# AlmondGod/diffusion-piano

Hardware: AMD Instinct MI355X
Metric: env steps/sec at 4096 parallel envs; qpos L∞ drift vs CPU MuJoCo (higher is better)
Workload: dtype f32; 1 GPU; 4096 envs/GPU crossing_field random-action rollout, 10 physics substeps per env-step, constraint forces by the primal Newton solve (friction loss, uncapped rows); envs_per_gpu=4096, song=crossing_field, parallelism=dp1

## Files before the change

diffusion-piano_amd/csrc/devmodel.h:

```cpp
#pragma once
#include <stdint.h>

#include "../../include/pianosim.h"

namespace ps {

constexpr int NK = PS_NKEY;
constexpr int NH = PS_NHAND;
constexpr int NB = PS_HAND_NBODY;
constexpr int ND = PS_HAND_NDOF;
constexpr int NG = PS_HAND_NGEOM;
constexpr int NA = PS_HAND_NACT;
constexpr int NV = PS_NV;
constexpr int NU = PS_NU;
constexpr int NBT = NH * NB;
constexpr int NDT = NH * ND;
constexpr int NGT = NH * NG;
constexpr int NX = PS_HAND_NXGEOM;
constexpr int NXT = NH * NX;
constexpr int NCOLL = NGT + NXT;
static_assert(NCOLL <= 64, "one lane per collider");
constexpr int NTT = NH * PS_HAND_NTENDON;
constexpr int MAXDEP = 9;
constexpr int MAXLEV = 8;
constexpr int MAXCHILD = 5;
constexpr int MAXCON = 24;
constexpr int KEYLANE = 52;
constexpr int YS = 20;
constexpr int YKEY = 19;
constexpr int NTRI = MAXDEP * (MAXDEP - 1) / 2;
constexpr int NKB = 64;
constexpr int KGEO = 16;
constexpr int XCG = 4;
constexpr int XNCELL = 6 * XCG * XCG;
constexpr int XCV = 8;

struct DevModel {
  float timestep;
  int nsub;
  float grav[3];
  float hgrav[3];
  float key_pos[NK][3], key_half[NK][3], key_anchor[NK][3];
  float key_mass[NK], key_Minv[NK], key_Mhinv[NK], key_damp[NK], key_stiff[NK], key_sref[NK];
  float key_lo[NK], key_hi[NK], key_ylo[NK], key_yhi[NK], key_binv[NK], key_dinv[NK];
  float base_pos[3], base_half[3];
  float pc_solref[2], pc_solimp[5], pc_fric;
  float hc_solref[2], hc_solimp[5], hc_fric;
  float lim_solref[2], lim_solimp[5];
  float fr_solref[2], fr_solimp[5];
  int body_parent[NBT];
  float body_pos[NBT][3], body_Q[NBT][9], body_mass[NBT], body_ipos[NBT][3], body_I[NBT][6];
  float body_binv[NBT];
  int body_dof[NBT], body_ndof[NBT];
  uint64_t body_pathmask[NBT];
  int nlev, lev_start[MAXLEV + 1], lev_body[NBT];
// ... 3 lines not shown
  float dof_floss[NDT];
  int dof_depth[NDT], dof_anc[NDT][MAXDEP];
  uint64_t dof_ancmask[NDT];
  uint64_t dof_descmask[NDT];
  int dof_ndesc[NDT], dof_desc[NDT][ND];
  int ndepth, dep_start[MAXDEP + 1], dep_dof[NDT];
  int dof_act[NDT];
  float dof_act_coef[NDT];
  int obs_dof[NDT];
  int n_obsj;
  uint64_t dof_lockmask;
  int act_src[NU];
  int n_action;
  int act_kind[NU], act_dof0[NU], act_dof1[NU], act_flim[NU];
  float act_c0[NU], act_c1[NU], act_kp[NU], act_clo[NU], act_chi[NU], act_flo[NU], act_fhi[NU];
  int geom_body[NCOLL];
  uint64_t geom_pathmask[NCOLL];
  float geom_binv[NCOLL];
  float geom_pos[NGT][3], geom_axis[NGT][3], geom_hl[NGT], geom_r[NGT];
  int root_geom_count;
  int site_body[NH * PS_NFINGER];
  float site_pos[NH * PS_NFINGER][3];
  int npairs;
  int pair[PS_MAX_CAPPAIRS][2];
  int nx;
  int x_type[NXT];
  float x_pos[NXT][3], x_Q[NXT][9], x_hs[NXT][3], x_rb[NXT];
  int x_v0[NXT], x_nv[NXT];
  float x_ec[NXT][8];
  uint64_t x_cell[NXT][XNCELL];
  alignas(16) float x_cellv[NXT][XNCELL + 1][XCV][4];
  int x_cellv_ok[NXT];
  int nxpairs;
  int nxpairs_same;
  int xpair[PS_MAX_XPAIRS];
  alignas(16) float hull_v[NH * PS_HAND_HULLVERT][4];
  int tri_a[NTRI + 8], tri_b[NTRI + 8];
  int body_level[NBT];
  int body_child_pack[NBT];
  int dof_anc_pack[NDT][3];
  float key_top_zmax;
  float piano_xmin, piano_xmax;
  float kb_y0, kb_inv;
  uint8_t kb_first[NKB], kb_end[NKB];
  int npairs_same;
  alignas(16) float key_geo[NK][KGEO];
};

}
```

diffusion-piano_amd/csrc/kernel_v2.inc:

```

#ifdef PS_TIMING
#define NPHASE 56
#define TARG , uint64_t *tacc, uint64_t &tlast
#define TPASS , tacc, tlast
#define TSTAMP(slot)                                     \
  do {                                                   \
    __syncthreads();                                     \
    uint64_t t_ = __builtin_amdgcn_s_memtime();         \
    tacc[slot] += t_ - tlast;                            \
    tlast = t_;                                          \
  } while (0)
__device__ uint64_t* g_timing = nullptr;
#else
#define TSTAMP(slot) \
  do {               \
  } while (0)
#define TARG
#define TPASS
#endif

#ifdef PS_CHECK_A
__device__ int g_dbg_count = 0;
#endif
enum : int { BX_R = 0, BX_CP = 0, BX_O = 10, BX_W = 13, BX_AL = 16, BX_AC = 19, BX_F = 22, BX_N = 25, BXS = 28 };
static_assert(NKB == 64, "collide2 stages one key-range bucket per lane");
// ... 381 lines not shown
        cc.g2 = g2;
      }
    }
  }
  return rt;
}

constexpr int NSTAGE = 32, STAGE_OFF = 2 * 256;
static_assert(STAGE_OFF >= 2 * NSTAGE, "candidate list overlaps the staging area");
constexpr int CPL = 8, CSTAGE_OFF = 2 * NGT * CPL;

template <bool XG, int WPE>
__device__ __forceinline__ int collide2(const DevModel* __restrict__ m, Shared& S, int maxc, int lane, float c_r TARG) {
  static_assert(STAGE_OFF + 2 * NSTAGE * sizeof(Contact) <= sizeof(S.bx), "contact staging exceeds bx");
  static_assert(CSTAGE_OFF + 2 * 64 * CPL <= sizeof(S.bx), "candidate staging exceeds bx");
  const bool isc = lane < NGT;
  {
    const float4* src = reinterpret_cast<const float4*>(&m->key_geo[0][0]);
    float4* dst = reinterpret_cast<float4*>(&S.kg[0][0]);
    for (int i = lane; i < NK * KGEO / 4; i += 64) dst[i] = src[i];
    S.kb[0][lane] = m->kb_first[lane];
    S.kb[1][lane] = m->kb_end[lane];
  }
  wsync();
  uint16_t* cand = reinterpret_cast<uint16_t*>(&S.bx[0][0]);
  constexpr int MAXCAND = (int)(sizeof(S.bx) / sizeof(uint16_t));
  int ncand;
  {
    uint16_t* cst = reinterpret_cast<uint16_t*>(reinterpret_cast<char*>(&S.bx[0][0]) + CSTAGE_OFF) + lane * CPL;
    const int cnt = isc ? piano_candidates(m, S, lane, c_r, cst, CPL) : 0;
    const int off = small_excl_scan<7>(cnt, lane, &ncand);
    if (__ballot(cnt > CPL) == 0ull) {
      for (int j = 0; j < cnt; j++) cand[off + j] = cst[j];
    } else if (isc && cnt && off + cnt <= MAXCAND) {
      piano_candidates(m, S, lane, c_r, cand + off, cnt);
    }
    ncand = min(ncand, MAXCAND);
  }
  wsync();
  TSTAMP(11);
  int total = 0;
  if (ncand <= NSTAGE) {
    Contact* stage = reinterpret_cast<Contact*>(reinterpret_cast<char*>(&S.bx[0][0]) + STAGE_OFF);
    const int pr = lane < ncand ? (int)cand[lane] : 0;
    const int cnt = lane < ncand ? piano_pair<WPE>(m, S, pr, stage, 2 * lane, 2 * lane + 2) : 0;
    int rt;
// ... 4 lines not shown
    ncand = 0;
  }
  for (int r0 = 0; r0 < ncand && total < maxc; r0 += 64) {
    const int i = r0 + lane;
    const int pr = i < ncand ? (int)cand[i] : 0;
    const int cnt = i < ncand ? piano_pair<WPE>(m, S, pr, nullptr, 0, 0) : 0;
    int rt;
    const int off = small_excl_scan<2>(cnt, lane, &rt);
    if (cnt) piano_pair<WPE>(m, S, pr, S.con, total + off, maxc);
    total += rt;
  }
  TSTAMP(7);
  int base = total;
  float lo[3], hi[3];
  {
    f3 p0 = isc ? ld3(&S.cap[lane][0]) : mk3(0, 0, 0), p1 = isc ? ld3(&S.cap[lane][3]) : mk3(0, 0, 0);
    lo[0] = fminf(p0.x, p1.x) - c_r; lo[1] = fminf(p0.y, p1.y) - c_r; lo[2] = fminf(p0.z, p1.z) - c_r;
    hi[0] = fmaxf(p0.x, p1.x) + c_r; hi[1] = fmaxf(p0.y, p1.y) + c_r; hi[2] = fmaxf(p0.z, p1.z) + c_r;
  }
  bool inb = isc;
  int hb = lane < NG ? 0 : 1;
  if (XG && lane >= NGT) {
    const int e = lane - NGT;
    inb = m->x_type[e] != PS_GEOM_NONE;
    hb = e / NX;
    if (inb) {
      const f3 ctr = ld3(S.xg[e]);
      const float rb = m->x_rb[e];
      lo[0] = ctr.x - rb; lo[1] = ctr.y - rb; lo[2] = ctr.z - rb;
      hi[0] = ctr.x + rb; hi[1] = ctr.y + rb; hi[2] = ctr.z + rb;
    }
  }
  bool apart = false;
  {
#pragma unroll
    for (int i = 0; i < 3; i++) {
      const float l0 = wave_min(inb && hb == 0 ? lo[i] : INFINITY), l1 = wave_min(inb && hb == 1 ? lo[i] : INFINITY);
      const float h0 = -wave_min(inb && hb == 0 ? -hi[i] : INFINITY),
                  h1 = -wave_min(inb && hb == 1 ? -hi[i] : INFINITY);
      if (h0 < l1 || h1 < l0) apart = true;
    }
  }
  const int npairs = apart ? m->npairs_same : m->npairs;
  uint16_t* near = cand;
  int nnear = 0;
  int pnext = lane < npairs ? m->pair[lane][0] | (m->pair[lane][1] << 8) : 0;
  for (int p0 = 0; p0 < npairs; p0 += 64) {
    const int p = p0 + lane;
    const int pk = pnext;
    if (p0 + 64 < npairs) pnext = p + 64 < npairs ? m->pair[p + 64][0] | (m->pair[p + 64][1] << 8) : 0;
    bool pass = false;
    if (p < npairs) {
      const float* A = S.cap[pk & 255];
      const float* B = S.cap[pk >> 8];
      const f3 ca = (ld3(A) + ld3(A + 3)) * 0.5f, cb = (ld3(B) + ld3(B + 3)) * 0.5f;
      pass = norm3(ca - cb) <= A[7] + B[7] + A[6] + B[6];
    }
    const uint64_t mask = __ballot(pass);
    if (pass) near[nnear + lanes_below(mask, lane)] = (uint16_t)pk;
    nnear += __popcll(mask);
  }
  wsync();
  for (int q0 = 0; q0 < nnear && base < maxc; q0 += 64) {
    const int q = q0 + lane;
    bool hit = false;
    f3 c1, c2;
    float ra = 0, rb = 0, dn = 0;
    int ga = 0, gb = 0;
    if (q < nnear) {
      const int pk = near[q];
      ga = pk & 255;
      gb = pk >> 8;
      const float* A = S.cap[ga];
      const float* B = S.cap[gb];
      ra = A[6];
      rb = B[6];
      seg_seg(ld3(A), ld3(A + 3), ld3(B), ld3(B + 3), &c1, &c2);
      dn = norm3(c2 - c1);
      hit = dn - ra - rb <= 0.f;
    }
    uint64_t mask = __ballot(hit);
    int slot = base + lanes_below(mask, lane);
    if (hit && slot < maxc) {
      Contact& cc = S.con[slot];
      f3 dv = c2 - c1;
      f3 n = dn > 1e-9f ? dv * (1.f / dn) : mk3(0, 0, 1);
      float dist = dn - ra - rb;
      st3(cc.n, n);
      cc.dist = dist;
      st3(cc.pos, c1 + n * (ra + 0.5f * dist));
      f3 t1, t2;
      make_frame(n, &t1, &t2);
      st3(cc.t1, t1); st3(cc.t2, t2);
      cc.kind = 2; cc.key = -1; cc.g1 = ga; cc.g2 = gb;
    }
    base += __popcll(mask);
  }
  if (XG && (m->nx || m->nxpairs)) {
    TSTAMP(2);
    int nl = 0;
    if (m->nx) {
      static_assert(NXT * CPL * 2 <= CSTAGE_OFF, "x candidates overlap the staging");
      const bool isx = lane >= NGT && m->x_type[lane >= NGT ? lane - NGT : 0] != PS_GEOM_NONE;
      uint16_t* cst = reinterpret_cast<uint16_t*>(reinterpret_cast<char*>(&S.bx[0][0]) + CSTAGE_OFF) + lane * CPL;
      wsync();
      const int cnt = isx ? xpiano_candidates(m, S, lane, cst, CPL) : 0;
      const int off = small_excl_scan<7>(cnt, lane, &nl);
      wsync();
      if (__ballot(cnt > CPL) == 0ull) {
        for (int j = 0; j < cnt; j++) cand[off + j] = cst[j];
      } else if (isx && cnt && off + cnt <= MAXCAND) {
        xpiano_candidates(m, S, lane, cand + off, cnt);
      }
      nl = min(nl, MAXCAND);
      wsync();
    }
    TSTAMP(32);
    if (m->nxpairs) {
      const int nxp = apart ? m->nxpairs_same : m->nxpairs;
      for (int p0 = 0; p0 < nxp; p0 += 64) {
        const int p = p0 + lane;
        bool pass = false;
        int pk = 0;
        if (p < nxp) {
          pk = m->xpair[p];
          const int ga = pk & 255, gb = pk >> 8;
          f3 c2[2];
          float rad = 0.f;
#pragma unroll
          for (int q = 0; q < 2; q++) {
            const int g = q ? gb : ga;
            if (g < NGT) {
              c2[q] = (ld3(&S.cap[g][0]) + ld3(&S.cap[g][3])) * 0.5f;
              rad += S.cap[g][6] + S.cap[g][7];
            } else {
              c2[q] = ld3(S.xg[g - NGT]);
              rad += m->x_rb[g - NGT];
            }
          }
          pass = norm3(c2[0] - c2[1]) <= rad;
        }
        const uint64_t mask = __ballot(pass);
        const int at = nl + lanes_below(mask, lane);
        if (pass && at < MAXCAND) cand[at] = (uint16_t)(pk | XHH);
        nl = min(nl + __popcll(mask), MAXCAND);
      }
#ifdef PS_TIMING
      tacc[45] += nl;
#endif
    }
    wsync();
    TSTAMP(35);
    nl = x_refine<WPE>(m, &S, cand, nl, lane);
#ifdef PS_TIMING
    tacc[42] += nl > 0;
#endif
    TSTAMP(36);
    for (int q0 = 0; q0 < nl && base < maxc; q0 += 32) {
      const int q = q0 + (lane >> 1);
      int ga, gb, key;
      x_entry(q < nl ? (int)cand[q] : 0, ga, gb, key);
#ifdef PS_TIMING
      int its[5] = {0, 0, 0, 0, 0};
      base += x_pairs<WPE>(m, &S, q < nl, ga, gb, key, S.con, base, maxc, lane, its);
      tacc[30] += its[0];
      tacc[31] += 1;
      tacc[38] += its[1];
      tacc[39] += its[2];
      tacc[40] += its[3];
      tacc[41] += its[4];
#else
      base += x_pairs<WPE>(m, &S, q < nl, ga, gb, key, S.con, base, maxc, lane);
#endif
    }
    TSTAMP(37);
  }
  if (lane == 0) S.ncon = base < maxc ? base : maxc;
  wsync();
  return base;
}

struct LaneStatic {
  int d_type, d_body, d_depth, d_ap0, d_ap1, d_act;
  uint64_t d_ancmask, d_desc;
  float d_axl[3], d_lo, d_hi, d_damp, d_arm, d_dinv, d_actc;
  bool d_lim;
  int b_parent, b_level, b_dof, b_ndof, b_chp, b_nch;
  int c_body;
  float c_r;
};

__device__ __forceinline__ void load_static(const DevModel* __restrict__ m, Shared& S, LaneStatic& L, int lane) {
  const int d = lane < NDT ? lane : 0, b = lane < NBT ? lane : 0, c = lane < NGT ? lane : 0;
  L.d_type = m->dof_type[d];
  L.d_body = m->dof_body[d];
  L.d_depth = lane < NDT ? m->dof_depth[d] : -1;
  L.d_ap0 = m->dof_anc_pack[d][0];
  L.d_ap1 = m->dof_anc_pack[d][1];
  L.d_act = m->dof_act[d];
  L.d_ancmask = m->dof_ancmask[d];
  L.d_desc = lane < NDT ? m->dof_descmask[d] : 0ull;
  for (int i = 0; i < 3; i++) L.d_axl[i] = m->dof_axis[d][i];
// ... 895 lines not shown
#pragma unroll
      for (int j = 0; j < 2; j++) {
        st_wt(pw + 64 * (CW_KQ + j), D.kq[j]);
        st_wt(pw + 64 * (CW_KV + j), D.kv[j]);
      }
      st_wt(pw + 64 * CW_CTRL, ctrl);
      st_wt(pw + 64 * CW_ACTF, actf_last);
      st_wt(pw + 64 * CW_ZF, __int_as_float(guess.zf));
      st_wt(pw + 64 * CW_ZL, __int_as_float(guess.zl));
      st_wt(pw + 64 * CW_ZC, __int_as_float(guess.zc));
      st_wt(pw + 64 * CW_CID, __int_as_float(guess.cid));
      st_wt(pw + 64 * CW_ZK, __int_as_float(guess.zk[0]));
      st_wt(pw + 64 * (CW_ZK + 1), __int_as_float(guess.zk[1]));
      const int sc = lane == CS_SOLVES ? st_solves : lane == CS_CONCAP ? st_concap : lane == CS_CAP ? st_cap
                   : lane == CS_MAXROW ? st_maxrow : lane == CS_COUPLED ? st_coupled : lane == CS_PIV ? st_piv
                   : lane == CS_CDOFS ? st_cdofs : lane == CS_WARN ? warn[0] : lane == CS_WARN + 1 ? warn[1]
                   : lane == CS_WARN + 2 ? warn[2] : lane == CS_GVALID ? (int)guess.valid
                   : (int)(bufs.applied && !applied);
      st_wt(pw + 64 * CW_SCAL, __int_as_float(sc));
      return true;
    }
  }
  kinematics2<false, XG>(m, S, L, D, lane, hand_dy TPASS);
  collide2<XG, WPE>(m, S, cfg.maxcon, lane, L.c_r TPASS);
  key_state2(m, S, D, lane);
  f3 root = mk3(0, 0, 0);
  if (cfg.hand) {
    const int B = (cfg.hand - 1) * NB;
    root = mk3(__shfl(D.o[0], B, 64), __shfl(D.o[1], B, 64), __shfl(D.o[2], B, 64));
  }
  if (do_reset) {
    write_obs2(m, song, cfg, S, 0, obs_e, lane, root);
    if (lane < NDT) {
      bufs.qpos[rowoff + NK + lane] = 0.f;
      bufs.qvel[rowoff + NK + lane] = 0.f;
      bufs.qws[rowoff + NK + lane] = 0.f;
    }
    for (int k = lane; k < NK; k += 64) {
      bufs.qpos[rowoff + k] = 0.f;
      bufs.qvel[rowoff + k] = 0.f;
      bufs.qws[rowoff + k] = 0.f;
    }
    if (lane < NU) bufs.ctrl[(size_t)e * NU + lane] = 0.f;
    if (lane < PS_NTERMS) bufs.terms[(size_t)e * PS_NTERMS + lane] = 0.f;
    if (lane < PS_NMUSIC) bufs.mus_acc[(size_t)e * PS_NMUSIC + lane] = 0.f;
    for (int s = 0; s < 2 * PS_NFINGER; s++) {
      f3 p = site_world2(m, D, s);
      if (lane == s) st3(bufs.tips + ((size_t)e * 2 * PS_NFINGER + s) * 3, p);
    }
    if (lane < PS_NSTATS) bufs.stats[(size_t)e * PS_NSTATS + lane] = 0;
    if (lane == 0) {
      bufs.sustain[e] = 0.f;
      bufs.t_idx[e] = 0;
      bufs.last[e] = 0;
      bufs.ncon[e] = S.ncon;
      if (bufs.keybits) bufs.keybits[(size_t)e * kb_stride(m->nsub)] = KB_NEW_EPISODE;
      if (mode == 0) {
        reward[e] = 0.f;
        discount[e] = 1.f;
        step_type[e] = PS_FIRST;
      }
    }
    return false;
  }
  const int t_cur = bufs.t_idx[e];
  const int t_new = t_cur + 1;
  const float* gc = song.goal + (size_t)t_cur * (NK + 1);
  float on_tol = 0.f, on_cnt = 0.f;
  bool fail_l = false;
  for (int k = lane; k < NK; k += 64) {
    float g = gc[k];
    bool act = (S.act_bits[k >> 5] >> (k & 31)) & 1;
    if (g != 0.f) { on_tol += tolerance(g - S.knorm[k], 0.f, 0.05f, 0.5f); on_cnt += 1.f; }
    else if (act) fail_l = true;
  }
  float sum_tol = wave_sum(on_tol), n_on = wave_sum(on_cnt);
  bool failure = __ballot(fail_l) != 0ull;
  float mus[PS_NMUSIC];
// ... 58 lines not shown
      if (on && pos < PS_MAX_NOTES) okeys[pos] = k;
      K += __popcll(mk);
    }
    K = min(K, PS_MAX_NOTES);
    wsync();
    float res = 1.f;
    if (K > 0) {
      for (int t0 = 0; t0 < 10 * K; t0 += 64) {
        const int t = t0 + lane;
        const int j = min(t / 10, K - 1), i = t - 10 * (t / 10);
        const int site = i < 5 ? PS_NFINGER + i : i - 5;
        const float tx = __shfl(tip_own.x, site, 64), ty = __shfl(tip_own.y, site, 64), tz = __shfl(tip_own.z, site, 64);
        const float dcost = norm3(key_target2(m, S, okeys[j]) - mk3(tx, ty, tz));
        if (t < 10 * K) ocost[K <= 10 ? j * 10 + i : i * K + j] = dcost < 1e30f ? dcost : 1e30f;
      }
      wsync();
      if (lane == 0) res = K <= 10 ? hungarian_tol(K, 10, ocost, owork) / K : hungarian_tol(10, K, ocost, owork) / 10.f;
    }
    fing = rdlane(res, 0);
  }
  float fore = 0.f;
  if (cfg.forearm) {
    bool hit = false;
    if (lane < S.ncon) {
      const Contact& cc = S.con[lane];
      if (cc.kind == 2) {
        const int b1 = m->geom_body[cc.g1], b2 = m->geom_body[cc.g2];
        hit = b1 % NB == 0 && b2 % NB == 0 && b1 != b2;
      }
    }
    fore = __ballot(hit) ? 0.f : 0.5f;
  }
  bool terminal = t_new == song.T;
  float disc = 1.f;
  if (!terminal && cfg.wrong_press && failure) { terminal = true; disc = 0.f; }
  write_obs2(m, song, cfg, S, t_new < song.T ? t_new : t_new - 1, obs_e, lane, root);
  if (lane < NDT) {
    bufs.qpos[rowoff + NK + lane] = D.q;
    bufs.qvel[rowoff + NK + lane] = D.v;
    bufs.qws[rowoff + NK + lane] = D.qws;
  }
#pragma unroll
  for (int j = 0; j < 2; j++) {
    int k = lane + 64 * j;
    if (k < NK) {
      bufs.qpos[rowoff + k] = D.kq[j];
      bufs.qvel[rowoff + k] = D.kv[j];
// ... 7 lines not shown
  if (lane < PS_NSTATS)
    bufs.stats[(size_t)e * PS_NSTATS + lane] = lane == 0 ? st_solves : lane == 1 ? st_concap : lane == 2 ? st_cap
                                               : lane == 3 ? st_maxrow : lane == 4 ? st_coupled
                                               : lane == 5 ? st_piv : st_cdofs;
  if (lane == 0) {
    float* tm = bufs.terms + (size_t)e * PS_NTERMS;
    tm[0] = kp; tm[1] = sus; tm[2] = energy; tm[3] = fing; tm[4] = fore;
    reward[e] = kp + sus + energy + fing + fore;
    discount[e] = disc;
    step_type[e] = terminal ? PS_LAST : PS_MID;
    float* ma = bufs.mus_acc + (size_t)e * PS_NMUSIC;
#pragma unroll
    for (int i = 0; i < PS_NMUSIC; i++) ma[i] += mus[i];
    if (terminal) {
      float* me = bufs.mus_ep + (size_t)e * PS_NMUSIC;
      const float inv = 1.f / (float)t_new;
#pragma unroll
      for (int i = 0; i < PS_NMUSIC; i++) me[i] = ma[i] * inv;
      bufs.mus_cnt[e] += 1;
    }
    bufs.sustain[e] = S.sustain;
    bufs.t_idx[e] = t_new;
    bufs.last[e] = terminal ? 1 : 0;
    bufs.ncon[e] = S.ncon;
    if (bufs.keybits) bufs.keybits[(size_t)e * kb_stride(m->nsub)] = (uint32_t)m->nsub;
  }
  if (bufs.con_out) {
    constexpr int CW = (int)(sizeof(Contact) / sizeof(int));
    const int* src = reinterpret_cast<const int*>(S.con);
    int* dst = reinterpret_cast<int*>(bufs.con_out) + (size_t)e * MAXCON * CW;
    for (int w = lane; w < S.ncon * CW; w += 64) dst[w] = src[w];
  }
#ifdef PS_TIMING
  TSTAMP(5);
  if (lane == 0 && g_timing)
    for (int i = 0; i < NPHASE; i++) g_timing[(size_t)e * NPHASE + i] += tacc[i];
#endif
  return false;
}

template <bool XG, int WPE = PS_WAVES_PER_EU>
__global__ void __launch_bounds__(64) __attribute__((amdgpu_waves_per_eu(WPE))) pianosim_kernel(const DevModel* __restrict__ m, Song song, Cfg cfg, Bufs bufs,
                                                      const float* __restrict__ action, const uint8_t* __restrict__ mask,
                                                      float* __restrict__ obs, float* __restrict__ reward,
                                                      float* __restrict__ discount, uint8_t* __restrict__ step_type,
                                                      int mode, int n_envs, const int* __restrict__ order) {
#ifdef PS_DYN_LDS
  extern __shared__ __attribute__((aligned(16))) char smem_[];
  Shared& S = *reinterpret_cast<Shared*>(smem_);
#else
  __shared__ Shared S;
#endif
  const int e = order ? order[blockIdx.x] : (int)blockIdx.x;
  const int lane = threadIdx.x;
  if (e >= n_envs) return;
  env_step<XG, WPE, false>(S, m, song, cfg, bufs, action, mask, obs, reward, discount, step_type, mode, e, lane, 0, 1);
}

enum : int { QC_HEAD = 0, QC_WORDS = 32 };
#ifndef PS_TIMING
enum : int { QE_NONE = -1, QE_LEFT = -2 };
struct QArgs {
  const DevModel* m;
  Song song;
  Cfg cfg;
  Bufs bufs;
  const float* action;
  float *obs, *reward, *discount;
  uint8_t* step_type;
  int n_envs;
  int *queue, *ctr;
  int cap, chunks;
  const int* rank;
#ifdef PS_QTRACE
  unsigned long long* trace;
#endif
};
enum : int { QT_ITEM = 4, QT_EXIT = 2 };
#ifdef PS_QTRACE
// ... 68 lines not shown
```

diffusion-piano_amd/csrc/model_build.h:

```cpp
#pragma once
#include <math.h>
#include <stdint.h>
#include <string.h>

#include <string>

#include "devmodel.h"

namespace ps {

inline int refuse(std::string& err, const std::string& s) { return err = s, -1; }

inline void quat2mat_h(const double* q, float* R) {
  double n = sqrt(q[0] * q[0] + q[1] * q[1] + q[2] * q[2] + q[3] * q[3]);
  double w = q[0] / n, x = q[1] / n, y = q[2] / n, z = q[3] / n;
  double M[9] = {1 - 2 * (y * y + z * z), 2 * (x * y - w * z), 2 * (x * z + w * y),
                 2 * (x * y + w * z), 1 - 2 * (x * x + z * z), 2 * (y * z - w * x),
                 2 * (x * z - w * y), 2 * (y * z + w * x), 1 - 2 * (x * x + y * y)};
  for (int i = 0; i < 9; i++) R[i] = (float)M[i];
}

inline void enclosing_capsule(const double (*v)[3], int n, float* out) {
  double best = INFINITY;
  double lo[3] = {INFINITY, INFINITY, INFINITY}, hi[3] = {-INFINITY, -INFINITY, -INFINITY};
// ... 417 lines not shown
    double y0 = m->key_ylo[0], y1 = m->key_yhi[NK - 1];
    for (int k = 0; k < NK; k++) { y0 = fmin(y0, m->key_ylo[k]); y1 = fmax(y1, m->key_yhi[k]); }
    double bw = (y1 - y0) / NKB;
    m->kb_y0 = (float)y0;
    m->kb_inv = (float)(1.0 / bw);
    for (int b = 0; b < NKB; b++) {
      double blo = y0 + b * bw, bhi = blo + bw;
      int f = 0;
      while (f < NK && m->key_yhi[f] < blo) f++;
      int e = f;
      while (e < NK && m->key_ylo[e] <= bhi) e++;
      m->kb_first[b] = (uint8_t)f;
      m->kb_end[b] = (uint8_t)e;
    }
  }
  for (int h = 0; h < NH; h++)
    for (int s = 0; s < PS_NFINGER; s++) {
      m->site_body[h * PS_NFINGER + s] = h * NB + d->site_body[h][s];
      for (int i = 0; i < 3; i++) m->site_pos[h * PS_NFINGER + s][i] = (float)d->site_pos[h][s][i];
    }
  if (d->n_cappairs < 0 || d->n_cappairs > PS_MAX_CAPPAIRS) return refuse(err, "bad n_cappairs");
  m->npairs = d->n_cappairs;
  for (int i = 0; i < d->n_cappairs; i++) {
    m->pair[i][0] = d->cappair[i][0];
    m->pair[i][1] = d->cappair[i][1];
    if (m->pair[i][0] < 0 || m->pair[i][0] >= NGT || m->pair[i][1] < 0 || m->pair[i][1] >= NGT)
      return refuse(err, "capsule pair index out of range");
    if (m->geom_r[m->pair[i][0]] < 0.f || m->geom_r[m->pair[i][1]] < 0.f) return refuse(err, "capsule pair names an unused slot");
  }
  m->npairs_same = 0;
  while (m->npairs_same < m->npairs && m->pair[m->npairs_same][0] / NG == m->pair[m->npairs_same][1] / NG)
    m->npairs_same++;
  for (int i = m->npairs_same; i < m->npairs; i++)
    if (m->pair[i][0] / NG == m->pair[i][1] / NG) { m->npairs_same = m->npairs; break; }
  auto xhand = [](int g) { return g < NGT ? g / NG : (g - NGT) / NX; };
  m->nxpairs_same = 0;
  while (m->nxpairs_same < m->nxpairs &&
         xhand(m->xpair[m->nxpairs_same] & 255) == xhand(m->xpair[m->nxpairs_same] >> 8))
    m->nxpairs_same++;
  for (int i = m->nxpairs_same; i < m->nxpairs; i++)
    if (xhand(m->xpair[i] & 255) == xhand(m->xpair[i] >> 8)) { m->nxpairs_same = m->nxpairs; break; }
  return 0;
}

inline int obs_dim(const ps_task_cfg* cfg, std::string& err) {
  if (!cfg || cfg->struct_size != PS_TASK_CFG_SIZE)
    return refuse(err, "ps_task_cfg.struct_size != sizeof(ps_task_cfg): rebuild against include/pianosim.h");
  if (cfg->hand_side != PS_HAND_BOTH)
    return (cfg->n_steps_lookahead + 1) * (NK + 1) + (cfg->fingering_reward ? 5 : 0) + NK + 1 + ND + 3;
  return (cfg->n_steps_lookahead + 1) * (NK + 1) + (cfg->fingering_reward ? 10 : 0) + NK + 1 + NH * ND;
}

inline int check_detached(const ps_model_desc* d, int h, std::string& err) {
  const std::string who = h ? "the left hand" : "the right hand";
  auto hand_of = [](int g) { return g < NGT ? g / NG : (g - NGT) / NX; };
  for (int j = 0; j < ND; j++)
    if (!d->dof_locked[h][j]) return refuse(err, "hand_side: " + who + " is not detached (dof " + std::to_string(j) + " is not locked)");
  for (int g = 0; g < NG; g++)
    if (d->geom_body[h][g] >= 0) return refuse(err, "hand_side: " + who + " is not detached (capsule " + std::to_string(g) + ")");
  for (int i = 0; i < NX; i++)
    if (d->xgeom_type[h][i] != PS_GEOM_NONE)
      return refuse(err, "hand_side: " + who + " is not detached (box / hull collider " + std::to_string(i) + ")");
  if (d->n_action <= 0) return refuse(err, "hand_side: " + who + " is not detached (the model has the full action row)");
  for (int a = 0; a < NA; a++)
// ... 49 lines not shown
```

diffusion-piano_amd/csrc/pianosim.hip:

```cpp
#include <hip/hip_runtime.h>
#include <math.h>
#include <stdint.h>
#include <stdio.h>
#include <stdlib.h>
#include <string.h>

#include <memory>
#include <string>
#include <vector>

#include "devmodel.h"
#include "model_build.h"
#include "prims.h"
#include "collide_x.h"

using namespace ps;

#include "kernel_v2.inc"
#include "augment.inc"
#include "midi_events.inc"

static thread_local std::string g_err;
static int fail(const std::string& s) {
  g_err = s;
// ... 42 lines not shown
  int *d_count, *d_keys, *d_fingers;
  float *qpos, *qvel, *qws, *ctrl, *sustain, *applied, *terms, *tips;
  int *t_idx, *ncon;
  float *mus_acc, *mus_ep;
  int* mus_cnt;
  int* order;
  bool ordered;
  uint8_t* last;
  bool applied_on;
  float* hand_dy;
  int* episode;
  int* stats;
  int* warnings;
  float* park;
  uint64_t seed;
  bool has_x;
  int wave_slots;
  int chunks, step_grid;
  bool chunks_forced;
  int *queue, *qctr;
  int* qrank;
  uint64_t* qtrace;
  Contact* con_out;
  bool aug_on;
  AugDev aug;
  size_t aug_lds;
  int nsub;
  uint32_t* keybits;
  MidiRec midi;
  DevMem mem, aug_mem, con_mem, midi_mem;
};

struct DeviceGuard {
  int prev = -1;
  bool ok = true;
  explicit DeviceGuard(int dev) {
    if (hipGetDevice(&prev) != hipSuccess) prev = -1;
    if (prev != dev) ok = hipSetDevice(dev) == hipSuccess;
  }
  ~DeviceGuard() {
    int cur = -1;
    if (prev >= 0 && hipGetDevice(&cur) == hipSuccess && cur != prev) (void)hipSetDevice(prev);
  }
};
#define GUARD(E)                                                                  \
  DeviceGuard guard_((E)->device);                                                \
// ... 162 lines not shown
    atomicAdd(&hist[b], 1);
  }
  __syncthreads();
  if (threadIdx.x == 0) {
    int acc = 0;
    for (int b = ORDER_BUCKETS - 1; b >= 0; b--) {
      base[b] = acc;
      acc += hist[b];
    }
  }
  __syncthreads();
  for (int e = threadIdx.x; e < n; e += blockDim.x) {
    const int b = last[e] ? 0 : 1 + min(max(stats[(size_t)e * PS_NSTATS + PS_STAT_SOLVES], 0), 128);
    const int pos = atomicAdd(&base[b], 1);
    if (queue) {
      queue[pos] = e << 4;
      qrank[e] = pos;
    } else {
      order[pos] = e;
    }
  }
}

static int launch(ps_env* E, int mode, const float* action, const uint8_t* mask, float* obs, float* reward,
                  float* discount, uint8_t* step_type, void* stream) {
  Song song{E->T, E->d_goal, E->d_count, E->d_keys, E->d_fingers, 0, nullptr};
  if (E->aug_on) {
    song = Song{E->T, E->aug.goal, E->aug.count, E->aug.keys, E->aug.fingers, E->aug.T_cap, E->aug.T};
    if (launch_builder(E, mode == 1 ? AUG_RESET : AUG_STEP, mask, nullptr, nullptr, nullptr, stream)) return -1;
  }
  Cfg cfg{};
  cfg.lookahead = E->cfg.n_steps_lookahead;
  cfg.fingering = E->cfg.fingering_reward;
  cfg.forearm = E->cfg.hand_side != PS_HAND_BOTH ? 0 : E->cfg.forearm_reward;
  cfg.wrong_press = E->cfg.wrong_press_termination;
  cfg.newton_cap = E->cfg.solver_iterations;
  cfg.maxcon = E->cfg.max_contacts;
  cfg.obs_dim = E->obs_dim;
  cfg.canonical = E->cfg.canonical_actions;
  cfg.energy_coef = (float)E->cfg.energy_penalty_coef;
  cfg.randomize = E->cfg.randomize_hand_positions != 0;
  cfg.seed_lo = (uint32_t)E->seed; cfg.seed_hi = (uint32_t)(E->seed >> 32);
  cfg.env0 = (uint32_t)E->env_offset;
  cfg.full_cpl = E->full_cpl;
  cfg.refine = E->cfg.solver_refine;
  cfg.hand = E->cfg.hand_side;
  Bufs b{};
  b.qpos = E->qpos; b.qvel = E->qvel; b.qws = E->qws; b.ctrl = E->ctrl; b.sustain = E->sustain;
  b.t_idx = E->t_idx; b.last = E->last; b.terms = E->terms; b.tips = E->tips; b.ncon = E->ncon;
  b.mus_acc = E->mus_acc; b.mus_ep = E->mus_ep; b.mus_cnt = E->mus_cnt; b.hand_dy = E->hand_dy;
  b.episode = E->episode; b.stats = E->stats; b.con_out = E->con_out; b.warnings = E->warnings; b.park = E->park;
  b.applied = E->applied_on ? E->applied : nullptr;
  b.keybits = E->keybits;
  const bool sliced = mode == 0 && E->chunks >= 2 &&
                      (E->chunks_forced || (E->n > E->step_grid && E->cfg.hand_side == PS_HAND_BOTH));
  if (sliced) {
    const int cap = E->n * E->chunks, grid = E->n < E->step_grid ? E->n : E->step_grid;
    hipLaunchKernelGGL(order_kernel, dim3(1), dim3(ORDER_THREADS), 0, (hipStream_t)stream, E->stats, E->last, E->order,
                       E->n, E->queue, E->qctr, cap, grid, E->ordered, E->qrank);
    HIPCHK(hipGetLastError());
#ifndef PS_TIMING
#ifdef PS_QTRACE
    HIPCHK(hipMemsetAsync(E->qtrace, 0, sizeof(uint64_t) * qtrace_words(E), (hipStream_t)stream));
    const QArgs qa{E->d_model, song, cfg, b, action, obs, reward, discount, step_type, E->n, E->queue, E->qctr, cap,
                   E->chunks, E->qrank, (unsigned long long*)E->qtrace};
#else
    const QArgs qa{E->d_model, song, cfg, b, action, obs, reward, discount, step_type, E->n, E->queue, E->qctr, cap,
                   E->chunks, E->qrank};
#endif
#define PS_LAUNCH_Q(XG)                                                                                           \
  hipLaunchKernelGGL((pianosim_queue_kernel<XG>), dim3(grid), dim3(64), 0, (hipStream_t)stream, qa)
    if (E->has_x) PS_LAUNCH_Q(true); else PS_LAUNCH_Q(false);
#undef PS_LAUNCH_Q
#endif
    HIPCHK(hipGetLastError());
    return E->keybits ? launch_midi(E, stream) : 0;
  }
  const int* order = nullptr;
  if (mode == 0 && E->ordered && E->n >= 2048) {
    hipLaunchKernelGGL(order_kernel, dim3(1), dim3(ORDER_THREADS), 0, (hipStream_t)stream, E->stats, E->last, E->order,
                       E->n, (int*)nullptr, (int*)nullptr, 0, 0, true, (int*)nullptr);
    HIPCHK(hipGetLastError());
    order = E->order;
  }
  const bool one = E->n <= E->wave_slots;
#define PS_LAUNCH(XG, WPE)                                                                                    \
  hipLaunchKernelGGL((pianosim_kernel<XG, WPE>), dim3(E->n), dim3(64), PS_LAUNCH_LDS, (hipStream_t)stream, \
                     E->d_model, song, cfg, b, action, mask, obs, reward, discount, step_type, mode, E->n, order)
  if (E->has_x) {
    if (one) PS_LAUNCH(true, 1); else PS_LAUNCH(true, PS_WAVES_PER_EU);
  } else {
    if (one) PS_LAUNCH(false, 1); else PS_LAUNCH(false, PS_WAVES_PER_EU);
  }
#undef PS_LAUNCH
  HIPCHK(hipGetLastError());
  return E->keybits ? launch_midi(E, stream) : 0;
}

int ps_reset(ps_env* E, const uint8_t* env_mask, float* obs, void* stream) {
  if (!E || !obs) return fail("null argument");
  GUARD(E);
  return launch(E, 1, nullptr, env_mask, obs, nullptr, nullptr, nullptr, stream);
}

int ps_step(ps_env* E, const float* action, float* obs, float* reward, float* discount, uint8_t* step_type,
            void* stream) {
  if (!E || !action || !obs || !reward || !discount || !step_type) return fail("null argument");
  GUARD(E);
  return launch(E, 0, action, nullptr, obs, reward, discount, step_type, stream);
}

int ps_get_state(ps_env* E, float* qpos, float* qvel, float* qacc_ws, float* ctrl, float* sustain, int32_t* t_idx,
                 uint8_t* last, void* stream) {
  if (!E) return fail("null env");
  GUARD(E);
  const size_t N = E->n;
  return -(copy_dd(qpos, E->qpos, N * NV, stream) || copy_dd(qvel, E->qvel, N * NV, stream) ||
           copy_dd(qacc_ws, E->qws, N * NV, stream) || copy_dd(ctrl, E->ctrl, N * NU, stream) ||
           copy_dd(sustain, E->sustain, N, stream) || copy_dd(t_idx, E->t_idx, N, stream) ||
           copy_dd(last, E->last, N, stream));
}

int ps_set_state(ps_env* E, const float* qpos, const float* qvel, const float* qacc_ws, const float* ctrl,
                 const float* sustain, const int32_t* t_idx, const uint8_t* last, void* stream) {
  if (!E) return fail("null env");
  GUARD(E);
  const size_t N = E->n;
  return -(copy_dd(E->qpos, qpos, N * NV, stream) || copy_dd(E->qvel, qvel, N * NV, stream) ||
           copy_dd(E->qws, qacc_ws, N * NV, stream) || copy_dd(E->ctrl, ctrl, N * NU, stream) ||
           copy_dd(E->sustain, sustain, N, stream) || copy_dd(E->t_idx, t_idx, N, stream) ||
           copy_dd(E->last, last, N, stream));
}

int ps_set_applied(ps_env* E, const float* qfrc_applied, void* stream) {
  if (!E) return fail("null env");
  GUARD(E);
  if (qfrc_applied && copy_dd(E->applied, qfrc_applied, (size_t)E->n * NV, stream)) return -1;
  E->applied_on = qfrc_applied != nullptr;
  return 0;
}

int ps_reward_terms(ps_env* E, float* terms, void* stream) {
  if (!E || !terms) return fail("null argument");
  GUARD(E);
  return copy_dd(terms, E->terms, (size_t)E->n * PS_NTERMS, stream);
}

int ps_fingertips(ps_env* E, float* xpos, void* stream) {
  if (!E || !xpos) return fail("null argument");
// ... 40 lines not shown
int ps_musical_metrics(ps_env* E, float* episode, int32_t* episodes, void* stream) {
  if (!E) return fail("null argument");
  GUARD(E);
  return -(copy_dd(episode, E->mus_ep, (size_t)E->n * PS_NMUSIC, stream) ||
           copy_dd(episodes, E->mus_cnt, (size_t)E->n, stream));
}

int ps_solver_stats(ps_env* E, int32_t* stats, void* stream) {
  if (!E || !stats) return fail("null argument");
  GUARD(E);
  return copy_dd(stats, E->stats, (size_t)E->n * PS_NSTATS, stream);
}

int ps_get_hand_offset(ps_env* E, float* dy, int32_t* episodes, void* stream) {
  if (!E) return fail("null argument");
  GUARD(E);
  return -(copy_dd(dy, E->hand_dy, (size_t)E->n, stream) || copy_dd(episodes, E->episode, (size_t)E->n, stream));
}

int ps_set_hand_offset(ps_env* E, const float* dy, void* stream) {
  if (!E || !dy) return fail("null argument");
  GUARD(E);
  if (!E->cfg.randomize_hand_positions) return fail("ps_set_hand_offset needs randomize_hand_positions");
  return copy_dd(E->hand_dy, dy, (size_t)E->n, stream);
}

static_assert(sizeof(ps_contact) == sizeof(Contact), "ps_contact mirrors the kernel's contact record");
int ps_record_contacts(ps_env* E, int on) {
  if (!E) return fail("null argument");
  GUARD(E);
  if (on && !E->con_out) {
    HIPCHK(E->con_mem.alloc(E->con_out, MAXCON * (size_t)E->n, true));
  } else if (!on && E->con_out) {
    E->con_mem.clear();
    E->con_out = nullptr;
  }
  return 0;
}

int ps_contacts(ps_env* E, ps_contact* out, void* stream) {
  if (!E || !out) return fail("null argument");
  GUARD(E);
  if (!E->con_out) return fail("contact recording is off (ps_record_contacts)");
  return copy_dd(reinterpret_cast<Contact*>(out), E->con_out, MAXCON * (size_t)E->n, stream);
}

// ... 218 lines not shown
      scnt[threadIdx.x] += scnt[threadIdx.x + w];
    }
    __syncthreads();
  }
  if (threadIdx.x == 0) {
    *finished_sum += ssum[0];
    *finished_count += scnt[0];
  }
}

int ps_episode_returns(const float* reward, const uint8_t* step_type, int n, double* running, float* last_return,
                       double* finished_sum, int64_t* finished_count, void* stream) {
  if (!reward || !step_type || !running || !last_return || !finished_sum || !finished_count || n <= 0)
    return fail("ps_episode_returns: null argument or n <= 0");
  hipLaunchKernelGGL(episode_returns_kernel, dim3(1), dim3(1024), 0, (hipStream_t)stream, reward, step_type, n, running,
                     last_return, finished_sum, finished_count);
  HIPCHK(hipGetLastError());
  return 0;
}

int ps_contact_count(ps_env* E, int32_t* ncon, void* stream) {
  if (!E || !ncon) return fail("null argument");
  GUARD(E);
  return copy_dd(ncon, E->ncon, (size_t)E->n, stream);
}

}
```

Measured before the change: 948,600 env-steps/s.

## Skip final post-step collision pass and compute contact counts lazily on demand

The end-of-step collide2 call, which only feeds the reported contact count and the forearm-hit term, is now skipped unless contacts are being recorded or a forearm pair's bounding volumes are close. Contact counts become stale and are recomputed by a new ncon kernel only when queried or before state is overwritten, with extra handling for graph capture. The pair list is also packed to uint16 and the pair broad-phase loops batch four loads per trip, and x_type/x_rb are hoisted into registers. This removes a full collision pass per env-step in the common case, at the cost of added bookkeeping complexity and a risk of stale ncon if the lazy paths are missed.

```diff
diff --git a/diffusion-piano_amd/csrc/devmodel.h b/diffusion-piano_amd/csrc/devmodel.h
--- a/diffusion-piano_amd/csrc/devmodel.h
+++ b/diffusion-piano_amd/csrc/devmodel.h
@@ -31,6 +31,7 @@
 constexpr int NTRI = MAXDEP * (MAXDEP - 1) / 2;
 constexpr int NKB = 64;
 constexpr int KGEO = 16;
+constexpr int MAXFORE = 64;
 constexpr int XCG = 4;
 constexpr int XNCELL = 6 * XCG * XCG;
 constexpr int XCV = 8;
@@ -80,7 +81,7 @@
   int site_body[NH * PS_NFINGER];
   float site_pos[NH * PS_NFINGER][3];
   int npairs;
-  int pair[PS_MAX_CAPPAIRS][2];
+  uint16_t pair[PS_MAX_CAPPAIRS];
   int nx;
   int x_type[NXT];
   float x_pos[NXT][3], x_Q[NXT][9], x_hs[NXT][3], x_rb[NXT];
@@ -103,6 +104,8 @@
   uint8_t kb_first[NKB], kb_end[NKB];
   int npairs_same;
   alignas(16) float key_geo[NK][KGEO];
+  int nfore;
+  uint16_t fore_pair[MAXFORE];
 };
 
 }
diff --git a/diffusion-piano_amd/csrc/kernel_v2.inc b/diffusion-piano_amd/csrc/kernel_v2.inc
--- a/diffusion-piano_amd/csrc/kernel_v2.inc
+++ b/diffusion-piano_amd/csrc/kernel_v2.inc
@@ -1,6 +1,7 @@
 
 #ifdef PS_TIMING
 #define NPHASE 56
+enum : int { TS_FINAL = 52, TS_FINAL_SKIP = 53 };
 #define TARG , uint64_t *tacc, uint64_t &tlast
 #define TPASS , tacc, tlast
 #define TSTAMP(slot)                                     \
@@ -428,6 +429,8 @@
     S.kb[0][lane] = m->kb_first[lane];
     S.kb[1][lane] = m->kb_end[lane];
   }
+  const int x_ty = XG ? m->x_type[lane >= NGT ? lane - NGT : 0] : (int)PS_GEOM_NONE;
+  const float x_rbl = XG ? m->x_rb[lane >= NGT ? lane - NGT : 0] : 0.f;
   wsync();
   uint16_t* cand = reinterpret_cast<uint16_t*>(&S.bx[0][0]);
   constexpr int MAXCAND = (int)(sizeof(S.bx) / sizeof(uint16_t));
@@ -478,11 +481,11 @@
   int hb = lane < NG ? 0 : 1;
   if (XG && lane >= NGT) {
     const int e = lane - NGT;
-    inb = m->x_type[e] != PS_GEOM_NONE;
+    inb = x_ty != PS_GEOM_NONE;
     hb = e / NX;
     if (inb) {
       const f3 ctr = ld3(S.xg[e]);
-      const float rb = m->x_rb[e];
+      const float rb = x_rbl;
       lo[0] = ctr.x - rb; lo[1] = ctr.y - rb; lo[2] = ctr.z - rb;
       hi[0] = ctr.x + rb; hi[1] = ctr.y + rb; hi[2] = ctr.z + rb;
     }
@@ -500,21 +503,26 @@
   const int npairs = apart ? m->npairs_same : m->npairs;
   uint16_t* near = cand;
   int nnear = 0;
-  int pnext = lane < npairs ? m->pair[lane][0] | (m->pair[lane][1] << 8) : 0;
-  for (int p0 = 0; p0 < npairs; p0 += 64) {
-    const int p = p0 + lane;
-    const int pk = pnext;
-    if (p0 + 64 < npairs) pnext = p + 64 < npairs ? m->pair[p + 64][0] | (m->pair[p + 64][1] << 8) : 0;
-    bool pass = false;
-    if (p < npairs) {
-      const float* A = S.cap[pk & 255];
-      const float* B = S.cap[pk >> 8];
-      const f3 ca = (ld3(A) + ld3(A + 3)) * 0.5f, cb = (ld3(B) + ld3(B + 3)) * 0.5f;
-      pass = norm3(ca - cb) <= A[7] + B[7] + A[6] + B[6];
-    }
-    const uint64_t mask = __ballot(pass);
-    if (pass) near[nnear + lanes_below(mask, lane)] = (uint16_t)pk;
-    nnear += __popcll(mask);
+  constexpr int PTRIPS = 4;
+  for (int p0 = 0; p0 < npairs; p0 += 64 * PTRIPS) {
+    int pks[PTRIPS];
+#pragma unroll
+    for (int u = 0; u < PTRIPS; u++) pks[u] = m->pair[min(p0 + 64 * u + lane, npairs - 1)];
+#pragma unroll
+    for (int u = 0; u < PTRIPS; u++) {
+      const int p = p0 + 64 * u + lane;
+      const int pk = pks[u];
+      bool pass = false;
+      if (p < npairs) {
+        const float* A = S.cap[pk & 255];
+        const float* B = S.cap[pk >> 8];
+        const f3 ca = (ld3(A) + ld3(A + 3)) * 0.5f, cb = (ld3(B) + ld3(B + 3)) * 0.5f;
+        pass = norm3(ca - cb) <= A[7] + B[7] + A[6] + B[6];
+      }
+      const uint64_t mask = __ballot(pass);
+      if (pass) near[nnear + lanes_below(mask, lane)] = (uint16_t)pk;
+      nnear += __popcll(mask);
+    }
   }
   wsync();
   for (int q0 = 0; q0 < nnear && base < maxc; q0 += 64) {
@@ -557,7 +565,7 @@
     int nl = 0;
     if (m->nx) {
       static_assert(NXT * CPL * 2 <= CSTAGE_OFF, "x candidates overlap the staging");
-      const bool isx = lane >= NGT && m->x_type[lane >= NGT ? lane - NGT : 0] != PS_GEOM_NONE;
+      const bool isx = lane >= NGT && x_ty != PS_GEOM_NONE;
       uint16_t* cst = reinterpret_cast<uint16_t*>(reinterpret_cast<char*>(&S.bx[0][0]) + CSTAGE_OFF) + lane * CPL;
       wsync();
       const int cnt = isx ? xpiano_candidates(m, S, lane, cst, CPL) : 0;
@@ -574,32 +582,38 @@
     TSTAMP(32);
     if (m->nxpairs) {
       const int nxp = apart ? m->nxpairs_same : m->nxpairs;
-      for (int p0 = 0; p0 < nxp; p0 += 64) {
-        const int p = p0 + lane;
-        bool pass = false;
-        int pk = 0;
-        if (p < nxp) {
-          pk = m->xpair[p];
+      for (int p0 = 0; p0 < nxp; p0 += 64 * PTRIPS) {
+        int pks[PTRIPS];
+#pragma unroll
+        for (int u = 0; u < PTRIPS; u++) pks[u] = m->xpair[min(p0 + 64 * u + lane, nxp - 1)];
+#pragma unroll
+        for (int u = 0; u < PTRIPS; u++) {
+          const int p = p0 + 64 * u + lane;
+          const int pk = pks[u];
           const int ga = pk & 255, gb = pk >> 8;
-          f3 c2[2];
-          float rad = 0.f;
-#pragma unroll
-          for (int q = 0; q < 2; q++) {
-            const int g = q ? gb : ga;
-            if (g < NGT) {
-              c2[q] = (ld3(&S.cap[g][0]) + ld3(&S.cap[g][3])) * 0.5f;
-              rad += S.cap[g][6] + S.cap[g][7];
-            } else {
-              c2[q] = ld3(S.xg[g - NGT]);
-              rad += m->x_rb[g - NGT];
+          const float rba = __shfl(x_rbl, ga, 64), rbb = __shfl(x_rbl, gb, 64);
+          bool pass = false;
+          if (p < nxp) {
+            f3 c2[2];
+            float rad = 0.f;
+#pragma unroll
+            for (int q = 0; q < 2; q++) {
+              const int g = q ? gb : ga;
+              if (g < NGT) {
+                c2[q] = (ld3(&S.cap[g][0]) + ld3(&S.cap[g][3])) * 0.5f;
+                rad += S.cap[g][6] + S.cap[g][7];
+              } else {
+                c2[q] = ld3(S.xg[g - NGT]);
+                rad += q ? rbb : rba;
+              }
             }
+            pass = norm3(c2[0] - c2[1]) <= rad;
           }
-          pass = norm3(c2[0] - c2[1]) <= rad;
+          const uint64_t mask = __ballot(pass);
+          const int at = nl + lanes_below(mask, lane);
+          if (pass && at < MAXCAND) cand[at] = (uint16_t)(pk | XHH);
+          nl = min(nl + __popcll(mask), MAXCAND);
         }
-        const uint64_t mask = __ballot(pass);
-        const int at = nl + lanes_below(mask, lane);
-        if (pass && at < MAXCAND) cand[at] = (uint16_t)(pk | XHH);
-        nl = min(nl + __popcll(mask), MAXCAND);
       }
 #ifdef PS_TIMING
       tacc[45] += nl;
@@ -634,6 +648,48 @@
   if (lane == 0) S.ncon = base < maxc ? base : maxc;
   wsync();
   return base;
+}
+
+template <bool XG>
+__device__ __forceinline__ bool fore_near(const DevModel* __restrict__ m, const Shared& S, int lane) {
+  const int nf = m->nfore;
+  if (nf < 0) return true;
+  bool pass = false;
+  if (lane < nf) {
+    const int pk = m->fore_pair[lane];
+    const int ga = pk & 255, gb = pk >> 8;
+    if (ga < NGT && gb < NGT) {
+      const float *A = S.cap[ga], *B = S.cap[gb];
+      const float reach = A[6] + B[6] + 1e-4f;
+      float d2 = 0.f;
+#pragma unroll
+      for (int i = 0; i < 3; i++) {
+        const float alo = fminf(A[i], A[3 + i]), ahi = fmaxf(A[i], A[3 + i]);
+        const float blo = fminf(B[i], B[3 + i]), bhi = fmaxf(B[i], B[3 + i]);
+        const float gap = fmaxf(0.f, fmaxf(alo - bhi, blo - ahi));
+        d2 += gap * gap;
+      }
+      pass = !(d2 > reach * reach);
+    } else if (XG) {
+      f3 c2[2];
+      float rad = 0.f;
+#pragma unroll
+      for (int q = 0; q < 2; q++) {
+        const int g = q ? gb : ga;
+        if (g < NGT) {
+          c2[q] = (ld3(&S.cap[g][0]) + ld3(&S.cap[g][3])) * 0.5f;
+          rad += S.cap[g][6] + S.cap[g][7];
+        } else {
+          c2[q] = ld3(S.xg[min(g - NGT, NXT - 1)]);
+          rad += m->x_rb[min(g - NGT, NXT - 1)];
+        }
+      }
+      pass = !(norm3(c2[0] - c2[1]) > rad * 1.00001f + 1e-6f);
+    } else {
+      pass = true;
+    }
+  }
+  return __ballot(pass) != 0ull;
 }
 
 struct LaneStatic {
@@ -1575,7 +1631,11 @@
     }
   }
   kinematics2<false, XG>(m, S, L, D, lane, hand_dy TPASS);
-  collide2<XG, WPE>(m, S, cfg.maxcon, lane, L.c_r TPASS);
+  const bool final_con = bufs.con_out != nullptr || (!do_reset && cfg.forearm && fore_near<XG>(m, S, lane));
+  if (final_con) collide2<XG, WPE>(m, S, cfg.maxcon, lane, L.c_r TPASS);
+#ifdef PS_TIMING
+  if (lane == 0 && !do_reset) { tacc[TS_FINAL] += 1; tacc[TS_FINAL_SKIP] += !final_con; }
+#endif
   key_state2(m, S, D, lane);
   f3 root = mk3(0, 0, 0);
   if (cfg.hand) {
@@ -1606,7 +1666,7 @@
       bufs.sustain[e] = 0.f;
       bufs.t_idx[e] = 0;
       bufs.last[e] = 0;
-      bufs.ncon[e] = S.ncon;
+      if (final_con) bufs.ncon[e] = S.ncon;
       if (bufs.keybits) bufs.keybits[(size_t)e * kb_stride(m->nsub)] = KB_NEW_EPISODE;
       if (mode == 0) {
         reward[e] = 0.f;
@@ -1711,7 +1771,7 @@
   float fore = 0.f;
   if (cfg.forearm) {
     bool hit = false;
-    if (lane < S.ncon) {
+    if (final_con && lane < S.ncon) {
       const Contact& cc = S.con[lane];
       if (cc.kind == 2) {
         const int b1 = m->geom_body[cc.g1], b2 = m->geom_body[cc.g2];
@@ -1765,7 +1825,7 @@
     bufs.sustain[e] = S.sustain;
     bufs.t_idx[e] = t_new;
     bufs.last[e] = terminal ? 1 : 0;
-    bufs.ncon[e] = S.ncon;
+    if (final_con) bufs.ncon[e] = S.ncon;
     if (bufs.keybits) bufs.keybits[(size_t)e * kb_stride(m->nsub)] = (uint32_t)m->nsub;
   }
   if (bufs.con_out) {
@@ -1798,6 +1858,35 @@
   const int lane = threadIdx.x;
   if (e >= n_envs) return;
   env_step<XG, WPE, false>(S, m, song, cfg, bufs, action, mask, obs, reward, discount, step_type, mode, e, lane, 0, 1);
+}
+
+template <bool XG>
+__global__ void __launch_bounds__(64) __attribute__((amdgpu_waves_per_eu(PS_WAVES_PER_EU))) pianosim_ncon_kernel(
+    const DevModel* __restrict__ m, Cfg cfg, Bufs bufs, int n_envs) {
+  __shared__ Shared S;
+  const int e = blockIdx.x, lane = threadIdx.x;
+  if (e >= n_envs) return;
+#ifdef PS_TIMING
+  uint64_t tacc[NPHASE] = {0};
+  uint64_t tlast = 0;
+#endif
+  LaneStatic L;
+  load_static(m, S, L, lane);
+  LaneDyn D;
+  const size_t rowoff = (size_t)e * NV;
+  D.v = 0.f;
+  D.q = bufs.qpos[rowoff + NK + (lane < NDT ? lane : 0)];
+#pragma unroll
+  for (int j = 0; j < 2; j++) {
+    const int k = lane + 64 * j;
+    D.kq[j] = bufs.qpos[rowoff + (k < NK ? k : 0)];
+    D.kv[j] = 0.f;
+  }
+  const float hand_dy = cfg.randomize ? bufs.hand_dy[e] : 0.f;
+  wsync();
+  kinematics2<false, XG>(m, S, L, D, lane, hand_dy TPASS);
+  collide2<XG, PS_WAVES_PER_EU>(m, S, cfg.maxcon, lane, L.c_r TPASS);
+  if (lane == 0) bufs.ncon[e] = S.ncon;
 }
 
 enum : int { QC_HEAD = 0, QC_WORDS = 32 };
diff --git a/diffusion-piano_amd/csrc/model_build.h b/diffusion-piano_amd/csrc/model_build.h
--- a/diffusion-piano_amd/csrc/model_build.h
+++ b/diffusion-piano_amd/csrc/model_build.h
@@ -463,17 +463,16 @@
   if (d->n_cappairs < 0 || d->n_cappairs > PS_MAX_CAPPAIRS) return refuse(err, "bad n_cappairs");
   m->npairs = d->n_cappairs;
   for (int i = 0; i < d->n_cappairs; i++) {
-    m->pair[i][0] = d->cappair[i][0];
-    m->pair[i][1] = d->cappair[i][1];
-    if (m->pair[i][0] < 0 || m->pair[i][0] >= NGT || m->pair[i][1] < 0 || m->pair[i][1] >= NGT)
-      return refuse(err, "capsule pair index out of range");
-    if (m->geom_r[m->pair[i][0]] < 0.f || m->geom_r[m->pair[i][1]] < 0.f) return refuse(err, "capsule pair names an unused slot");
-  }
+    const int a = d->cappair[i][0], b = d->cappair[i][1];
+    if (a < 0 || a >= NGT || b < 0 || b >= NGT) return refuse(err, "capsule pair index out of range");
+    if (m->geom_r[a] < 0.f || m->geom_r[b] < 0.f) return refuse(err, "capsule pair names an unused slot");
+    m->pair[i] = (uint16_t)(a | (b << 8));
+  }
+  auto same_hand = [m](int i) { return (m->pair[i] & 255) / NG == (m->pair[i] >> 8) / NG; };
   m->npairs_same = 0;
-  while (m->npairs_same < m->npairs && m->pair[m->npairs_same][0] / NG == m->pair[m->npairs_same][1] / NG)
-    m->npairs_same++;
+  while (m->npairs_same < m->npairs && same_hand(m->npairs_same)) m->npairs_same++;
   for (int i = m->npairs_same; i < m->npairs; i++)
-    if (m->pair[i][0] / NG == m->pair[i][1] / NG) { m->npairs_same = m->npairs; break; }
+    if (same_hand(i)) { m->npairs_same = m->npairs; break; }
   auto xhand = [](int g) { return g < NGT ? g / NG : (g - NGT) / NX; };
   m->nxpairs_same = 0;
   while (m->nxpairs_same < m->nxpairs &&
@@ -481,6 +480,15 @@
     m->nxpairs_same++;
   for (int i = m->nxpairs_same; i < m->nxpairs; i++)
     if (xhand(m->xpair[i] & 255) == xhand(m->xpair[i] >> 8)) { m->nxpairs_same = m->nxpairs; break; }
+  m->nfore = 0;
+  auto fore = [m](int a, int b) {
+    const int ba = m->geom_body[a], bb = m->geom_body[b];
+    if (ba % NB != 0 || bb % NB != 0 || ba == bb || m->nfore < 0) return;
+    if (m->nfore == MAXFORE) { m->nfore = -1; return; }
+    m->fore_pair[m->nfore++] = (uint16_t)(a | (b << 8));
+  };
+  for (int i = 0; i < m->npairs; i++) fore(m->pair[i] & 255, m->pair[i] >> 8);
+  for (int i = 0; i < m->nxpairs; i++) fore(m->xpair[i] & 255, m->xpair[i] >> 8);
   return 0;
 }
 
diff --git a/diffusion-piano_amd/csrc/pianosim.hip b/diffusion-piano_amd/csrc/pianosim.hip
--- a/diffusion-piano_amd/csrc/pianosim.hip
+++ b/diffusion-piano_amd/csrc/pianosim.hip
@@ -88,6 +88,7 @@
   int* qrank;
   uint64_t* qtrace;
   Contact* con_out;
+  bool ncon_stale, ncon_sticky;
   bool aug_on;
   AugDev aug;
   size_t aug_lds;
@@ -296,13 +297,7 @@
   }
 }
 
-static int launch(ps_env* E, int mode, const float* action, const uint8_t* mask, float* obs, float* reward,
-                  float* discount, uint8_t* step_type, void* stream) {
-  Song song{E->T, E->d_goal, E->d_count, E->d_keys, E->d_fingers, 0, nullptr};
-  if (E->aug_on) {
-    song = Song{E->T, E->aug.goal, E->aug.count, E->aug.keys, E->aug.fingers, E->aug.T_cap, E->aug.T};
-    if (launch_builder(E, mode == 1 ? AUG_RESET : AUG_STEP, mask, nullptr, nullptr, nullptr, stream)) return -1;
-  }
+static Cfg make_cfg(const ps_env* E) {
   Cfg cfg{};
   cfg.lookahead = E->cfg.n_steps_lookahead;
   cfg.fingering = E->cfg.fingering_reward;
@@ -319,6 +314,10 @@
   cfg.full_cpl = E->full_cpl;
   cfg.refine = E->cfg.solver_refine;
   cfg.hand = E->cfg.hand_side;
+  return cfg;
+}
+
+static Bufs make_bufs(const ps_env* E) {
   Bufs b{};
   b.qpos = E->qpos; b.qvel = E->qvel; b.qws = E->qws; b.ctrl = E->ctrl; b.sustain = E->sustain;
   b.t_idx = E->t_idx; b.last = E->last; b.terms = E->terms; b.tips = E->tips; b.ncon = E->ncon;
@@ -326,6 +325,49 @@
   b.episode = E->episode; b.stats = E->stats; b.con_out = E->con_out; b.warnings = E->warnings; b.park = E->park;
   b.applied = E->applied_on ? E->applied : nullptr;
   b.keybits = E->keybits;
+  return b;
+}
+
+static bool capturing(void* stream) {
+  hipStreamCaptureStatus cs = hipStreamCaptureStatusNone;
+  if (hipStreamIsCapturing((hipStream_t)stream, &cs) != hipSuccess) {
+    (void)hipGetLastError();
+    return false;
+  }
+  return cs != hipStreamCaptureStatusNone;
+}
+
+static int materialise_ncon(ps_env* E, void* stream) {
+  const bool cap = capturing(stream);
+  if (!E->ncon_stale && !E->ncon_sticky && !cap) return 0;
+  const Cfg cfg = make_cfg(E);
+  const Bufs b = make_bufs(E);
+  if (E->has_x)
+    hipLaunchKernelGGL((pianosim_ncon_kernel<true>), dim3(E->n), dim3(64), 0, (hipStream_t)stream,
+                       E->d_model, cfg, b, E->n);
+  else
+    hipLaunchKernelGGL((pianosim_ncon_kernel<false>), dim3(E->n), dim3(64), 0, (hipStream_t)stream,
+                       E->d_model, cfg, b, E->n);
+  HIPCHK(hipGetLastError());
+  if (!cap) E->ncon_stale = false;
+  return 0;
+}
+
+static void mark_ncon(ps_env* E, void* stream) {
+  if (E->con_out) return;
+  E->ncon_stale = true;
+  if (capturing(stream)) E->ncon_sticky = true;
+}
+
+static int launch(ps_env* E, int mode, const float* action, const uint8_t* mask, float* obs, float* reward,
+                  float* discount, uint8_t* step_type, void* stream) {
+  Song song{E->T, E->d_goal, E->d_count, E->d_keys, E->d_fingers, 0, nullptr};
+  if (E->aug_on) {
+    song = Song{E->T, E->aug.goal, E->aug.count, E->aug.keys, E->aug.fingers, E->aug.T_cap, E->aug.T};
+    if (launch_builder(E, mode == 1 ? AUG_RESET : AUG_STEP, mask, nullptr, nullptr, nullptr, stream)) return -1;
+  }
+  const Cfg cfg = make_cfg(E);
+  const Bufs b = make_bufs(E);
   const bool sliced = mode == 0 && E->chunks >= 2 &&
                       (E->chunks_forced || (E->n > E->step_grid && E->cfg.hand_side == PS_HAND_BOTH));
   if (sliced) {
@@ -348,6 +390,7 @@
 #undef PS_LAUNCH_Q
 #endif
     HIPCHK(hipGetLastError());
+    mark_ncon(E, stream);
     return E->keybits ? launch_midi(E, stream) : 0;
   }
   const int* order = nullptr;
@@ -368,6 +411,7 @@
   }
 #undef PS_LAUNCH
   HIPCHK(hipGetLastError());
+  mark_ncon(E, stream);
   return E->keybits ? launch_midi(E, stream) : 0;
 }
 
@@ -399,6 +443,7 @@
                  const float* sustain, const int32_t* t_idx, const uint8_t* last, void* stream) {
   if (!E) return fail("null env");
   GUARD(E);
+  if (materialise_ncon(E, stream)) return -1;
   const size_t N = E->n;
   return -(copy_dd(E->qpos, qpos, N * NV, stream) || copy_dd(E->qvel, qvel, N * NV, stream) ||
            copy_dd(E->qws, qacc_ws, N * NV, stream) || copy_dd(E->ctrl, ctrl, N * NU, stream) ||
@@ -485,6 +530,7 @@
   if (!E || !dy) return fail("null argument");
   GUARD(E);
   if (!E->cfg.randomize_hand_positions) return fail("ps_set_hand_offset needs randomize_hand_positions");
+  if (materialise_ncon(E, stream)) return -1;
   return copy_dd(E->hand_dy, dy, (size_t)E->n, stream);
 }
 
@@ -749,6 +795,7 @@
 int ps_contact_count(ps_env* E, int32_t* ncon, void* stream) {
   if (!E || !ncon) return fail("null argument");
   GUARD(E);
+  if (materialise_ncon(E, stream)) return -1;
   return copy_dd(ncon, E->ncon, (size_t)E->n, stream);
 }
 
```

Result: faster. 963,900 env-steps/s, median of 6 (+1.6%).
